# permon/permon

Measured on NVIDIA B200. Metric: mpgp_iterations_per_second, higher is better.
Workload: dtype f64

## Files before the change

### permon_b200/csrc/kernels.cu

```cuda
#include <climits>
#include <cuda_runtime.h>
#include <nvtx3/nvToolsExt.h>
#include <stdarg.h>
#include <stddef.h>
#include <stdio.h>
#include <string.h>
#include <time.h>

#include <algorithm>
#include <string>
#include <type_traits>
#include <utility>
#include <vector>

#include "device.h"

namespace pb {

static DevCtx      g_ctx;
int                g_p2p_size = 1;
static std::string g_err;
DevCtx            &ctx() { return g_ctx; }
const char        *last_error() { return g_err.c_str(); }

// ... 1137 lines not shown
  if (warp == PK_CT / 32) {
    int pidn = 0;
    if (blockIdx.x < ntiles) pidn = __ldg(A.st_pid + tile_at(blockIdx.x, ord.ta, ord.tb, rev));
    int      s = 0, filled = 0;
    uint32_t ph = 0;
    for (int i = blockIdx.x; i < ntiles; i += gridDim.x) {
      const int tile = tile_at(i, ord.ta, ord.tb, rev);
      const int pid = pidn;
      const int ni = i + gridDim.x;
      if (ni < ntiles) pidn = __ldg(A.st_pid + tile_at(ni, ord.ta, ord.tb, rev));
      if (filled >= nstages) mbar_wait(&empty_bar[s], ph ^ 1u);
      else filled++;
      unsigned char   *st = stages + (size_t)s * stage_bytes;
      const StPattern *P = reinterpret_cast<const StPattern *>(smem_raw) + pid;
      const int        r0 = tile * TR, r1 = min(r0 + TR, A.n);
      const bool       fullt = (r1 - r0 == TR) && vec_tma;
      bool             windowed = fullt && win_ok;
      uint32_t         wbytes = 0;
      const int        nwin = P->nwin;
      for (int w = 0; w < nwin; w++) {
        const int lo = r0 + P->wlo[w];
        if (lo < 0 || lo + P->wlen[w] > A.ncols) windowed = false;
        wbytes += (uint32_t)P->wlen[w] * 8u;
      }
      if (lane == 0) {
        reinterpret_cast<int *>(st)[0] = pid;
        reinterpret_cast<int *>(st)[1] = windowed ? 1 : 0;
      }
      if (fullt) {
        if (lane == 0) {
          mbar_arrive_expect_tx(&full_bar[s], (uint32_t)TR + (uint32_t)nv * TR * 8u + (windowed ? wbytes : 0u));
          bulk_g2s(st + ST_MASK_OFF, A.st_masks + r0, (uint32_t)TR, &full_bar[s]);
          if (windowed)
            for (int w = 0; w < nwin; w++) bulk_g2s(st + ST_WIN_OFF + (size_t)w * PB_ST_WCAP, x + (r0 + P->wlo[w]), (uint32_t)P->wlen[w] * 8u, &full_bar[s]);
          for (int v = 0; v < nv; v++) bulk_g2s(st + vec_off + (size_t)v * TR * 8, epi.vsrc(v) + r0, (uint32_t)TR * 8u, &full_bar[s]);
        }
      } else {
        for (int t = lane; t < TR; t += 32) st[ST_MASK_OFF + t] = (t < r1 - r0) ? __ldg(A.st_masks + r0 + t) : (unsigned char)0;
        for (int v = 0; v < nv; v++) {
          double       *vs = (double *)(st + vec_off) + (size_t)v * TR;
          const double *src = epi.vsrc(v) + r0;
          for (int t = lane; t < r1 - r0; t += 32) vs[t] = src[t];
        }
        fence_proxy_async_smem();
        __syncwarp();
        if (lane == 0) mbar_arrive(&full_bar[s]);
      }
      if (++s == nstages) {
        s = 0;
        ph ^= 1u;
      }
    }
  } else {
    const uint32_t smem_a = smem_u32(smem_raw), stages_a = smem_a + (uint32_t)pats_bytes;
    int            s = 0;
    uint32_t       ph = 0;
    for (int i = blockIdx.x; i < ntiles; i += gridDim.x) {
      const int tile = tile_at(i, ord.ta, ord.tb, rev);
      mbar_wait(&full_bar[s], ph);
      const uint32_t st_a = stages_a + (uint32_t)s * (uint32_t)stage_bytes;
      const uint32_t vs_a = st_a + (uint32_t)vec_off + 8u * threadIdx.x;
      const uint32_t pid = (uint32_t)lds_s32(st_a), windowed = (uint32_t)lds_s32(st_a + 4u);
      const uint32_t P_a = smem_a + pid * (uint32_t)sizeof(StPattern);
      const uint32_t L = (uint32_t)lds_s32(P_a);
      const uint32_t m0 = lds_u8(st_a + ST_MASK_OFF + threadIdx.x), m1 = lds_u8(st_a + ST_MASK_OFF + threadIdx.x + PK_CT);
      const int      r0 = tile * TR + threadIdx.x, r1 = r0 + PK_CT;
      double         s0, s1;
      if (windowed) st_win2_dispatch(L, m0, m1, P_a, st_a + ST_WIN_OFF + 8u * threadIdx.x, gx, s0, s1);
      else st_row2_dispatch(L, m0, m1, P_a + (uint32_t)offsetof(StPattern, v), P_a + (uint32_t)offsetof(StPattern, d), gx, r0, r1, s0, s1);
      if (r0 < A.n) epi.row_s(r0, vs_a, s0, acc);
      if (r1 < A.n) epi.row_s(r1, vs_a + PK_CT * 8u, s1, acc);
      __syncwarp();
      if (lane == 0) mbar_arrive(&empty_bar[s]);
      if (++s == nstages) {
        s = 0;
        ph ^= 1u;
      }
    }
  }
  epi.finalize(acc);
}


template <int LMAX, class G>
__device__ __forceinline__ double sd_row(int L, uint32_t m, const StPattern &P, const G &gx, int r)
{
  constexpr uint32_t FULL = (1u << LMAX) - 1u;
  const char        *xr = reinterpret_cast<const char *>(gx.x + r);
  if (__all_sync(0xffffffffu, L == LMAX && m == FULL)) {
    double xv[LMAX];
    int    db[LMAX];
#pragma unroll
    for (int j = 0; j < LMAX; j++) db[j] = P.d[j] * 8;
#pragma unroll
    for (int j = 0; j < LMAX; j++) xv[j] = gx.ld(reinterpret_cast<const double *>(xr + (long long)db[j]));
    __syncwarp();
    double s = 0.0;
#pragma unroll
    for (int j = 0; j < LMAX; j++) s += P.v[j] * xv[j];
    return s;
  }
  double xv[LMAX], vv[LMAX];
#pragma unroll
  for (int j = 0; j < LMAX; j++) {
    const bool on = (j < L) && ((m >> j) & 1u);
    xv[j]         = on ? gx.ld(reinterpret_cast<const double *>(xr + (long long)(P.d[j] * 8))) : 0.0;
  }
  __syncwarp();
#pragma unroll
  for (int j = 0; j < LMAX; j++) vv[j] = P.v[j];
  double s = 0.0;
#pragma unroll
  for (int j = 0; j < LMAX; j++)
    if ((j < L) && ((m >> j) & 1u)) s += vv[j] * xv[j];
  return s;
}

__device__ __forceinline__ void l2_prefetch_bulk(const double *p, long long e0, long long e1, long long n)
{
  if (e0 < 0) e0 = 0;
  if (e1 > n) e1 = n;
  uintptr_t a0 = (uintptr_t)(p + e0), a1 = (uintptr_t)(p + e1);
  a0 = (a0 + 15) & ~(uintptr_t)15;
  a1 &= ~(uintptr_t)15;
  if (a1 > a0) asm volatile("cp.async.bulk.prefetch.L2.global [%0], %1;" ::"l"(a0), "r"((uint32_t)(a1 - a0)) : "memory");
}
template <class Epi>
__device__ __forceinline__ void sd_prefetch_tile(const Epi &epi, const double *gx, int tile, int rows, int n, int ncols, bool rev, const TileOrder &ord, int lane)
{
  const long long r0 = (long long)tile * rows;
  const int       nv = epi.nvec();
  if (lane == 0) {
    const int d = rev ? ord.dlo : ord.dhi;
    l2_prefetch_bulk(gx, r0 + d, r0 + d + rows, ncols);
  } else if (lane <= nv) {
    const double *v = epi.vsrc(lane - 1);
    if (v != gx) l2_prefetch_bulk(v, r0, r0 + rows, n);
  }
}

template <class Epi, int LMAX, int MINB>
__global__ void __launch_bounds__(NT, MINB) k_spmv_sd(CsrDev A, const double *__restrict__ x, Epi epi, TileOrder ord)
{
  pdl_enter();
  if (!epi.active()) return;
  __shared__ StPattern s_pats[PB_ST_MAXPAT];
  {
    const int  nw = A.st_npat * (int)(sizeof(StPattern) / 4);
    const int *src = reinterpret_cast<const int *>(A.st_pats);
    int       *dst = reinterpret_cast<int *>(s_pats);
    for (int k = threadIdx.x; k < nw; k += NT) dst[k] = __ldg(src + k);
  }
  __syncthreads();
  const int  ntiles = (A.n + TR - 1) / TR;
  const bool rev = epi.reverse();
  const typename Epi::Gather gx = epi.gather(x);
  typename Epi::Acc acc;
  epi.init(acc);
  uint32_t m_next = 0;
  int      pid_next = 0;
  if ((int)blockIdx.x < ntiles) {
    const int t0 = tile_at(blockIdx.x, ord.ta, ord.tb, rev);
    pid_next = __ldg(A.st_pid + t0);
    m_next   = __ldg(A.st_masks + (size_t)t0 * TR + threadIdx.x);
  }
  for (int i = blockIdx.x; i < ntiles; i += gridDim.x) {
    const int      tile = tile_at(i, ord.ta, ord.tb, rev);
    const uint32_t m = m_next;
    const int      pid = pid_next;
    const int      ni = i + gridDim.x;
    const int      r = tile * TR + threadIdx.x;
    const bool     live = r < A.n;
    if (ord.pf > 0 && threadIdx.x < 32) {
      const long long pi = (long long)i + (long long)ord.pf * gridDim.x;
      if (pi < ntiles) sd_prefetch_tile(epi, gx.x, tile_at((int)pi, ord.ta, ord.tb, rev), TR, A.n, A.ncols, rev, ord, (int)threadIdx.x);
    }
    const typename Epi::Pre pre = epi.preload(live ? r : 0);
    if (ni < ntiles) {
      const int tn = tile_at(ni, ord.ta, ord.tb, rev);
      pid_next = __ldg(A.st_pid + tn);
      m_next   = __ldg(A.st_masks + (size_t)tn * TR + threadIdx.x);
    }
    const StPattern &P = s_pats[pid];
    const double     sum = sd_row<LMAX>(P.L, m, P, gx, r);
    if (live) epi.row_p(r, sum, pre, acc);
  }
  epi.finalize(acc);
}


template <int LMAX, class G>
__device__ __forceinline__ void sd_row2(int L, uint32_t m0, uint32_t m1, const StPattern &P, const G &gx, int r, double &s0, double &s1)
{
  constexpr uint32_t FULL = (1u << LMAX) - 1u;
  const char        *xr = reinterpret_cast<const char *>(gx.x + r);
  double             x0[LMAX], x1[LMAX], vv[LMAX];
  if (__all_sync(0xffffffffu, L == LMAX && m0 == FULL && m1 == FULL)) {
#pragma unroll
    for (int j = 0; j < LMAX; j++) {
      const double *a = reinterpret_cast<const double *>(xr + (long long)(P.d[j] * 8));
      x0[j]           = gx.ld(a);
      x1[j]           = gx.ld(a + 1);
    }
    __syncwarp();
#pragma unroll
    for (int j = 0; j < LMAX; j++) vv[j] = P.v[j];
    s0 = 0.0;
    s1 = 0.0;
#pragma unroll
    for (int j = 0; j < LMAX; j++) s0 += vv[j] * x0[j];
#pragma unroll
    for (int j = 0; j < LMAX; j++) s1 += vv[j] * x1[j];
    return;
  }
#pragma unroll
  for (int j = 0; j < LMAX; j++) {
    const double *a = reinterpret_cast<const double *>(xr + (long long)(P.d[j] * 8));
    const bool    on0 = (j < L) && ((m0 >> j) & 1u), on1 = (j < L) && ((m1 >> j) & 1u);
    x0[j]             = on0 ? gx.ld(a) : 0.0;
    x1[j]             = on1 ? gx.ld(a + 1) : 0.0;
  }
  __syncwarp();
#pragma unroll
  for (int j = 0; j < LMAX; j++) vv[j] = P.v[j];
  s0 = 0.0;
  s1 = 0.0;
#pragma unroll
  for (int j = 0; j < LMAX; j++)
    if ((j < L) && ((m0 >> j) & 1u)) s0 += vv[j] * x0[j];
#pragma unroll
  for (int j = 0; j < LMAX; j++)
    if ((j < L) && ((m1 >> j) & 1u)) s1 += vv[j] * x1[j];
}

template <class Epi, int LMAX, int MINB>
__global__ void __launch_bounds__(NT, MINB) k_spmv_sd2(CsrDev A, const double *__restrict__ x, Epi epi, TileOrder ord)
{
  pdl_enter();
  if (!epi.active()) return;
  __shared__ StPattern s_pats[PB_ST_MAXPAT];
  {
    const int  nw = A.st_npat * (int)(sizeof(StPattern) / 4);
    const int *src = reinterpret_cast<const int *>(A.st_pats);
    int       *dst = reinterpret_cast<int *>(s_pats);
    for (int k = threadIdx.x; k < nw; k += NT) dst[k] = __ldg(src + k);
  }
  __syncthreads();
  const int  nst = (A.n + 2 * TR - 1) / (2 * TR);
  const int  half = threadIdx.x >> 7;
  const bool rev = epi.reverse();
  const typename Epi::Gather gx = epi.gather(x);
  typename Epi::Acc acc;
  epi.init(acc);
  uchar2 m_next = make_uchar2(0, 0);
  int    pid_next = 0;
  if ((int)blockIdx.x < nst) {
    const int t0 = tile_at(blockIdx.x, ord.ta, ord.tb, rev);
    pid_next = __ldg(A.st_pid + 2 * t0 + half);
    m_next   = __ldg(reinterpret_cast<const uchar2 *>(A.st_masks + (size_t)t0 * (2 * TR)) + threadIdx.x);
  }
  for (int i = blockIdx.x; i < nst; i += gridDim.x) {
    const int    st = tile_at(i, ord.ta, ord.tb, rev);
    const uchar2 m = m_next;
    const int    pid = pid_next;
    const int    ni = i + gridDim.x;
    const int    r = st * (2 * TR) + 2 * (int)threadIdx.x;
    const bool   live = r < A.n;
    const typename Epi::Pre2 pre = epi.preload2(live ? r : 0);
// ... 276 lines not shown
    }
    static size_t attr_smem = 0;
    if (smem > attr_smem) {
      cudaFuncSetAttribute(k_spmv_st<Epi>, cudaFuncAttributeMaxDynamicSharedMemorySize, (int)smem);
      attr_smem = smem;
    }
    static int    occ = 0;
    static size_t occ_smem = (size_t)-1;
    if (!occ || occ_smem != smem) {
      int nb = 0;
      if (cudaOccupancyMaxActiveBlocksPerMultiprocessor(&nb, k_spmv_st<Epi>, PK_CT + 32, smem) != cudaSuccess || nb < 1) nb = 1;
      occ      = nb;
      occ_smem = smem;
    }
    int ntiles = (A.n + TR - 1) / TR, grid = g_ctx.sm_count * occ;
    if (grid > ntiles) grid = ntiles;
    if (grid > max_red_blocks()) grid = max_red_blocks();
    if (ord.tb <= ord.ta || ord.tb > ntiles) {
      ord.ta = 0;
      ord.tb = ntiles;
    }
    launch_k(k_spmv_st<Epi>, grid, PK_CT + 32, smem, A, x, epi, nstages, (int)stage, pats_bytes, win_ok, vec_tma, ord);
    return 0;
  }
}


template <class Epi, int LMAX>
static int launch_sd_l(const CsrDev &A, const double *x, const Epi &epi, TileOrder ord)
{
  static int pairs = -1;
  if (pairs < 0) {
    const char *e = getenv("PERMON_B200_SD_PAIRS");
    pairs = (e && e[0] == '1') ? 1 : 0;
  }
  if (pairs && (A.n % 2 == 0) && aligned16(x) && epi.pair_ok()) {
    auto       k2 = k_spmv_sd2<Epi, LMAX, 4>;
    static int occ2 = 0;
    if (!occ2) {
      int nb = 0;
      if (cudaOccupancyMaxActiveBlocksPerMultiprocessor(&nb, k2, NT, 0) != cudaSuccess || nb < 1) nb = 1;
      occ2 = nb;
    }
    const int ntiles = (A.n + TR - 1) / TR, nst = (ntiles + 1) / 2;
    int       grid = g_ctx.sm_count * occ2;
    if (grid > nst) grid = nst;
    if (grid > max_red_blocks()) grid = max_red_blocks();
    TileOrder o2;
    o2.ta = (ord.ta + 1) / 2;
    o2.tb = ord.tb / 2;
    if (o2.tb <= o2.ta || o2.tb > nst || ord.tb <= ord.ta || ord.tb > ntiles || (ord.ta == 0 && ord.tb == ntiles)) {
      o2.ta = 0;
      o2.tb = nst;
    }
    launch_k(k2, grid, NT, 0, A, x, epi, o2);
    return 0;
  }
  auto kern = k_spmv_sd<Epi, LMAX, 5>;
  static int pf = -1;
  if (pf < 0) {
    const char *e = getenv("PERMON_B200_SD_PF");
    pf = e ? atoi(e) : 0;
    if (pf < 0 || pf > 64) pf = 0;
  }
  ord.pf  = pf;
  ord.dlo = A.st_dlo;
  ord.dhi = A.st_dhi;
  static int occ = 0;
  if (!occ) {
    int nb = 0;
    if (cudaOccupancyMaxActiveBlocksPerMultiprocessor(&nb, kern, NT, 0) != cudaSuccess || nb < 1) nb = 1;
    occ = nb;
  }
  int ntiles = (A.n + TR - 1) / TR, grid = g_ctx.sm_count * occ;
  if (grid > ntiles) grid = ntiles;
  if (grid > max_red_blocks()) grid = max_red_blocks();
  if (ord.tb <= ord.ta || ord.tb > ntiles) {
    ord.ta = 0;
    ord.tb = ntiles;
  }
  launch_k(kern, grid, NT, 0, A, x, epi, ord);
  return 0;
}
template <class Epi>
static int launch_sd(const CsrDev &A, const double *x, const Epi &epi, TileOrder ord)
{
  switch (A.st_lmax) {
  case 3: return launch_sd_l<Epi, 3>(A, x, epi, ord);
  case 5: return launch_sd_l<Epi, 5>(A, x, epi, ord);
  case 7: return launch_sd_l<Epi, 7>(A, x, epi, ord);
  default: return launch_sd_l<Epi, 8>(A, x, epi, ord);
  }
}

template <class Epi>
static int launch_spmv(const CsrDev &A, const double *x, const Epi &epi, int family, double bytes, TileOrder ord = TileOrder())
{
  prof_pre(family, bytes);
  if (A.n == 0) {
    k_spmv_vector<Epi, 32><<<1, NT, 0, g_ctx.stream>>>(A, x, epi);
  } else if (A.kind == 5) {
    launch_ell(A, x, epi);
  } else if (A.kind == 4) {
    static int direct = -1;
    if (direct < 0) {
      const char *e = getenv("PERMON_B200_ST_KERNEL");
      direct = (e && !strcmp(e, "windows")) ? 0 : 1;
    }
    if (direct) PB_CHK(launch_sd(A, x, epi, ord));
    else PB_CHK(launch_st(A, x, epi, ord));
  } else if (A.kind == 3) {
    PB_CHK(launch_pk(A, x, epi, ord));
  } else if (A.kind == 2) {
    launch_tma(A, x, epi);
  } else if (A.kind == 0) {
    static int    occ = 0;
    static size_t occ_smem = (size_t)-1;
    size_t        smem = (size_t)A.tile_cap * sizeof(double);
    if (!occ || occ_smem != smem) {
      occ      = occ_blocks(k_spmv_stream<Epi>, smem);
      occ_smem = smem;
    }
    int ntiles = (A.n + TR - 1) / TR;
    int grid   = g_ctx.sm_count * occ;
    if (grid > ntiles) grid = ntiles;
    if (grid > max_red_blocks()) grid = max_red_blocks();
    k_spmv_stream<Epi><<<grid, NT, smem, g_ctx.stream>>>(A, x, epi);
  } else {
    switch (A.W) {
    case 2: launch_vector<Epi, 2>(A, x, epi); break;
    case 4: launch_vector<Epi, 4>(A, x, epi); break;
    case 8: launch_vector<Epi, 8>(A, x, epi); break;
    case 16: launch_vector<Epi, 16>(A, x, epi); break;
    default: launch_vector<Epi, 32>(A, x, epi); break;
    }
  }
  prof_post(family);
  LAUNCH_CHECK();
  return 0;
}

double csr_stream_bytes(const CsrDev &A)
{
  if (A.kind == 3 || A.kind == 4) return (double)A.pk_bytes;
  if (A.kind == 5) return 12.0 * (double)A.ell_elems + 4.0 * A.n;
  return 12.0 * (double)A.nnz + 4.0 * (A.n + 1);
}

void spmv_stats(int n, const int *h_ia, int *maxrow_out, int *cap_out)
{
  int maxrow = 0, cap = 0;
  for (int r0 = 0; r0 < n; r0 += TR) {
    int r1 = (r0 + TR < n) ? r0 + TR : n;
    int t  = h_ia[r1] - h_ia[r0];
    if (t > cap) cap = t;
  }
#pragma omp parallel for reduction(max : maxrow) schedule(static)
  for (int r = 0; r < n; r++) {
    int l = h_ia[r + 1] - h_ia[r];
    if (l > maxrow) maxrow = l;
  }
  *maxrow_out = maxrow;
  *cap_out    = cap;
}
int spmv_config(CsrDev &A, const int *h_ia)
{
  int maxrow, cap;
  spmv_stats(A.n, h_ia, &maxrow, &cap);
  spmv_decide(A, maxrow, cap);
  return 0;
}
void spmv_decide(CsrDev &A, int maxrow, int cap)
{
  const int n = A.n;
  const double avg = n ? (double)A.nnz / n : 0.0;
  const char  *force = getenv("PERMON_B200_SPMV");
  bool         stream = (cap <= 5632 && maxrow <= 64);
  if (force && !strcmp(force, "vector")) stream = false;
  if (stream) {
    A.kind     = 2;
    if ((force && !strcmp(force, "stream")) || A.rows) A.kind = 0;
    A.tile_cap = (cap + 3 + 31) & ~31;
    if (A.tile_cap < 32) A.tile_cap = 32;
    const char *st = getenv("PERMON_B200_STAGES");
    A.stages = st ? atoi(st) : 2;
  } else {
    A.kind = 1;
    int W  = 32;
    if (avg <= 3) W = 2;
    else if (avg <= 6) W = 4;
    else if (avg <= 12) W = 8;
    else if (avg <= 24) W = 16;
    A.W = W;
  }
}

struct EpiPlain {
  typedef GatherPlain Gather;
  __device__ Gather gather(const double *x) const { return Gather{x}; }
  double *y;
  int     accumulate;
  struct Acc {};
  __device__ bool active() const { return true; }
  __device__ bool reverse() const { return false; }
  __device__ void init(Acc &) const {}
  __device__ void row(int r, double ax, Acc &) const { y[r] = accumulate ? y[r] + ax : ax; }
  struct Pre {};
  __device__ Pre preload(int) const { return Pre{}; }
  __device__ void row_p(int r, double ax, const Pre &, Acc &a) const { row(r, ax, a); }
  __device__ void finalize(Acc &) const {}
  __host__ __device__ int  nvec() const { return 0; }
  __host__ __device__ const double *vsrc(int) const { return nullptr; }
  int nvec_host() const { return nvec(); }
  const double *vsrc_host(int i) const { return vsrc(i); }
  __device__ void row_s(int r, uint32_t, double ax, Acc &a) const { row(r, ax, a); }

  struct Pre2 {};
  __device__ Pre2 preload2(int) const { return Pre2{}; }
  __device__ void row2_p(int r, double a0, double a1, const Pre2 &, Acc &a) const
  {
    row(r, a0, a);
    row(r + 1, a1, a);
  }
  bool pair_ok() const { return true; }
};

struct EpiGated {
  typedef GatherPlain Gather;
  __device__ Gather gather(const double *x) const { return Gather{x}; }
  double        *y;
  const MpgpCtl *S;
  int            phase;
  struct Acc {};
  __device__ bool active() const
  {
    if (S->reason != 0) return false;
    return phase == 0 ? true : (S->step == 'e' || S->init);
  }
  __device__ bool reverse() const { return false; }
  __device__ void init(Acc &) const {}
  __device__ void row(int r, double ax, Acc &) const { y[r] = ax; }
  struct Pre {};
  __device__ Pre preload(int) const { return Pre{}; }
  __device__ void row_p(int r, double ax, const Pre &, Acc &a) const { row(r, ax, a); }
  struct Pre2 {};
  __device__ Pre2 preload2(int) const { return Pre2{}; }
  __device__ void row2_p(int r, double a0, double a1, const Pre2 &, Acc &a) const
  {
    row(r, a0, a);
    row(r + 1, a1, a);
  }
  bool pair_ok() const { return true; }
  __device__ void finalize(Acc &) const {}
  __host__ __device__ int  nvec() const { return 0; }
  __host__ __device__ const double *vsrc(int) const { return nullptr; }
  int nvec_host() const { return nvec(); }
  const double *vsrc_host(int i) const { return vsrc(i); }
  __device__ void row_s(int r, uint32_t, double ax, Acc &a) const { row(r, ax, a); }
};

struct AccRed {
  double v[PB_NRED];
  int    halo_ok;
};

struct GhostRet {
  double ax;
  int    ok;
};
__device__ __noinline__ GhostRet ghost_slow(const GhostMerge &gm, int r, double ax, int halo_ok)
{
  GhostRet  out{ax, halo_ok};
  const int k = __ldg(gm.row_map + (r < gm.lo ? r : r - gm.hi + gm.lo));
  if (k < 0) return out;
  if (!halo_ok) {
    for (int q = 0; q < gm.nflags; q++) wait_flag(gm.flags + (size_t)q * PB_FLAG_STRIDE, gm.seq);
    out.ok = 1;
  }
  const int e0 = __ldg(gm.oia + k), e1 = __ldg(gm.oia + k + 1);
  for (int e = e0; e < e1; e++) out.ax += __ldg(gm.oa + e) * __ldcg(gm.ghost + __ldg(gm.oja + e));
  return out;
}
__device__ __forceinline__ double ghost_apply(const GhostMerge &gm, int r, double ax, int &halo_ok)
{
  if (gm.row_map == nullptr || (r >= gm.lo && r < gm.hi)) return ax;
  const GhostRet g = ghost_slow(gm, r, ax, halo_ok);
  halo_ok = g.ok;
  return g.ax;
}

template <int MODE, bool GHOST>
struct EpiAT {
  typedef GatherPlain Gather;
  __device__ Gather gather(const double *x) const { return Gather{x}; }
  const double        *p, *x;
  double              *Ap;
  BoxDev               bx;
  const double        *B;
  int                  m, n;
  const MpgpCtl       *S;
  RedBuf               rb;
  GhostMerge           gm;
  typedef AccRed       Acc;
  __device__ bool active() const { return S->reason == 0; }
  __device__ bool reverse() const { return S->sweep != 0; }
  __device__ void init(Acc &a) const
  {
#pragma unroll
    for (int k = 0; k < PB_NRED; k++) a.v[k] = 0.0;
    a.v[RA_FEAS] = HUGE_VAL;
    a.halo_ok    = 0;
  }
  __device__ void row(int r, double ax, Acc &a) const
  {
    if constexpr (GHOST) ax = ghost_apply(gm, r, ax, a.halo_ok);
    Ap[r] = ax;
    const double pr = __ldg(p + r);
    a.v[RA_PAP] += pr * ax;
    if constexpr (MODE != 0) {
      BoxVal b;
      b.has_lb = true;
      b.has_ub = (MODE == 2);
      b.lb     = __ldg(bx.lb + r);
      b.ub     = (MODE == 2) ? __ldg(bx.ub + r) : 0.0;
      a.v[RA_FEAS] = box_feas_lazy(__ldg(x + r), pr, b, a.v[RA_FEAS]);
    } else {
#pragma unroll
      for (int j = 0; j < PB_MAXEQ; j++)
        if (j < m) a.v[RA_BP + j] += B[(size_t)j * n + r] * pr;
      a.v[RA_FEAS] = box_feas_lazy(x[r], pr, load_box(bx, r), a.v[RA_FEAS]);
    }
  }
  struct Pre {
    double p, x, lb, ub;
  };
  __device__ Pre preload(int r) const
  {
    Pre q;
    q.p  = __ldg(p + r);
    q.x  = __ldg(x + r);
    q.lb = (MODE != 0 || bx.lb) ? __ldg(bx.lb + r) : 0.0;
    q.ub = (MODE == 2 || (MODE == 0 && bx.ub)) ? __ldg(bx.ub + r) : 0.0;
    return q;
  }
  __device__ void row_p(int r, double ax, const Pre &q, Acc &a) const
  {
    if constexpr (GHOST) ax = ghost_apply(gm, r, ax, a.halo_ok);
    Ap[r] = ax;
    a.v[RA_PAP] += q.p * ax;
    BoxVal b;
    b.has_lb = (MODE != 0) || bx.lb != nullptr;
    b.has_ub = (MODE == 2) || (MODE == 0 && bx.ub != nullptr);
    b.lb     = q.lb;
    b.ub     = q.ub;
    if constexpr (MODE == 0) {
#pragma unroll
      for (int j = 0; j < PB_MAXEQ; j++)
        if (j < m) a.v[RA_BP + j] += B[(size_t)j * n + r] * q.p;
    }
    a.v[RA_FEAS] = box_feas_lazy(q.x, q.p, b, a.v[RA_FEAS]);
  }
  struct Pre2 {
    double2 p, x, lb, ub;
  };
  __device__ Pre2 preload2(int r) const
  {
    Pre2 q;
    q.p  = __ldg(reinterpret_cast<const double2 *>(p + r));
    q.x  = __ldg(reinterpret_cast<const double2 *>(x + r));
    q.lb = (MODE != 0 || bx.lb) ? __ldg(reinterpret_cast<const double2 *>(bx.lb + r)) : make_double2(0.0, 0.0);
    q.ub = (MODE == 2 || (MODE == 0 && bx.ub)) ? __ldg(reinterpret_cast<const double2 *>(bx.ub + r)) : make_double2(0.0, 0.0);
    return q;
  }
  __device__ void row2_p(int r, double a0, double a1, const Pre2 &q, Acc &a) const
  {
    if constexpr (GHOST) {
      a0 = ghost_apply(gm, r, a0, a.halo_ok);
      a1 = ghost_apply(gm, r + 1, a1, a.halo_ok);
    }
    *reinterpret_cast<double2 *>(Ap + r) = make_double2(a0, a1);
    a.v[RA_PAP] += q.p.x * a0;
    a.v[RA_PAP] += q.p.y * a1;
    BoxVal b0, b1;
    b0.has_lb = b1.has_lb = (MODE != 0) || bx.lb != nullptr;
    b0.has_ub = b1.has_ub = (MODE == 2) || (MODE == 0 && bx.ub != nullptr);
    b0.lb = q.lb.x; b1.lb = q.lb.y;
    b0.ub = q.ub.x; b1.ub = q.ub.y;
    if constexpr (MODE == 0) {
#pragma unroll
      for (int j = 0; j < PB_MAXEQ; j++)
        if (j < m) {
          a.v[RA_BP + j] += B[(size_t)j * n + r] * q.p.x;
          a.v[RA_BP + j] += B[(size_t)j * n + r + 1] * q.p.y;
        }
    }
    a.v[RA_FEAS] = box_feas_lazy(q.x.x, q.p.x, b0, a.v[RA_FEAS]);
    a.v[RA_FEAS] = box_feas_lazy(q.x.y, q.p.y, b1, a.v[RA_FEAS]);
  }
  bool pair_ok() const { return aligned16(p) && aligned16(x) && aligned16(Ap) && aligned16(bx.lb) && aligned16(bx.ub); }
  __device__ void finalize(Acc &a) const { grid_reduce8<(1 << RA_FEAS)>(a.v, rb, nullptr); }
  __host__ __device__ int nvec() const { return 2 + (bx.lb ? 1 : 0) + (bx.ub ? 1 : 0) + m; }
  int nvec_host() const { return nvec(); }
  const double *vsrc_host(int i) const { return vsrc(i); }
  __host__ __device__ const double *vsrc(int i) const
  {
    if (i == 0) return p;
    if (i == 1) return x;
    int k = 2;
    if (bx.lb) {
      if (i == k) return bx.lb;
      k++;
    }
    if (bx.ub) {
      if (i == k) return bx.ub;
      k++;
    }
    return B + (size_t)(i - k) * n;
  }
  __device__ void row_s(int r, uint32_t va, double ax, Acc &a) const
  {
    if constexpr (GHOST) ax = ghost_apply(gm, r, ax, a.halo_ok);
    Ap[r] = ax;
    const double pr = lds_f64(va);
    a.v[RA_PAP] += pr * ax;
    const double xr = lds_f64(va + TR * 8);
    if constexpr (MODE != 0) {
      BoxVal b;
      b.has_lb = true;
      b.has_ub = (MODE == 2);
      b.lb     = lds_f64(va + 2 * TR * 8);
      b.ub     = (MODE == 2) ? lds_f64(va + 3 * TR * 8) : 0.0;
      a.v[RA_FEAS] = box_feas_lazy(xr, pr, b, a.v[RA_FEAS]);
    } else {
      BoxVal   b;
      uint32_t k = 2;
      b.has_lb = bx.lb != nullptr;
      b.has_ub = bx.ub != nullptr;
      b.lb     = b.has_lb ? lds_f64(va + (k++) * TR * 8) : 0.0;
      b.ub     = b.has_ub ? lds_f64(va + (k++) * TR * 8) : 0.0;
#pragma unroll
      for (int j = 0; j < PB_MAXEQ; j++)
        if (j < m) a.v[RA_BP + j] += lds_f64(va + (k + j) * TR * 8) * pr;
      a.v[RA_FEAS] = box_feas_lazy(xr, pr, b, a.v[RA_FEAS]);
    }
  }
};

template <int MODE, bool GHOST>
struct EpiA2T {
  typedef GatherPlain Gather;
  __device__ Gather gather(const double *x) const { return Gather{x}; }
  const double        *x, *b;
  double              *g, *p;
  BoxDev               bx;
  const double        *B;
  int                  m, n;
  const MpgpCtl       *S;
  RedBuf               rb;
  GhostMerge           gm;
  typedef AccRed       Acc;
  __device__ bool active() const { return S->reason == 0 && (S->step == 'e' || S->init); }
  __device__ bool reverse() const { return S->sweep != 0; }
  __device__ void init(Acc &a) const
  {
#pragma unroll
    for (int k = 0; k < PB_NRED; k++) a.v[k] = 0.0;
    a.halo_ok = 0;
  }
  __device__ void row(int r, double ax, Acc &a) const
  {
    double gr = ax;
    if constexpr (GHOST) gr = ghost_apply(gm, r, ax, a.halo_ok);
    BoxVal bv;
    if constexpr (MODE != 0) {
      bv.has_lb = true;
      bv.has_ub = (MODE == 2);
      bv.lb     = __ldg(bx.lb + r);
      bv.ub     = (MODE == 2) ? __ldg(bx.ub + r) : 0.0;
    } else {
      bv = load_box(bx, r);
      if (m > 0) {
        double t = 0.0;
        for (int j = 0; j < m; j++) t += B[(size_t)j * n + r] * S->Bu[j];
        gr += S->rho * t;
      }
    }
    gr -= __ldg(b + r);
    double gf, gc;
    box_split(x[r], gr, bv, bx.astol, gf, gc);
    g[r] = gr;
    p[r] = gf;
    const double gP = gf + gc;
    a.v[RB_GP2] += gP * gP;
    a.v[RB_GC2] += gc * gc;
    a.v[RB_GF2] += gf * gf;
  }
  struct Pre {
    double x, b, lb, ub;
  };
  __device__ Pre preload(int r) const
  {
    Pre q;
    q.x  = __ldg(x + r);
    q.b  = __ldg(b + r);
    q.lb = (MODE != 0 || bx.lb) ? __ldg(bx.lb + r) : 0.0;
    q.ub = (MODE == 2 || (MODE == 0 && bx.ub)) ? __ldg(bx.ub + r) : 0.0;
    return q;
  }
  __device__ void row_p(int r, double ax, const Pre &q, Acc &a) const
  {
    double gr = ax;
    if constexpr (GHOST) gr = ghost_apply(gm, r, ax, a.halo_ok);
    BoxVal bv;
    bv.has_lb = (MODE != 0) || bx.lb != nullptr;
    bv.has_ub = (MODE == 2) || (MODE == 0 && bx.ub != nullptr);
    bv.lb     = q.lb;
    bv.ub     = q.ub;
    if constexpr (MODE == 0) {
      if (m > 0) {
        double t = 0.0;
        for (int j = 0; j < m; j++) t += B[(size_t)j * n + r] * S->Bu[j];
        gr += S->rho * t;
      }
    }
    gr -= q.b;
    double gf, gc;
    box_split(q.x, gr, bv, bx.astol, gf, gc);
    g[r] = gr;
    p[r] = gf;
    const double gP = gf + gc;
    a.v[RB_GP2] += gP * gP;
    a.v[RB_GC2] += gc * gc;
    a.v[RB_GF2] += gf * gf;
// ... 26 lines not shown
      if (m > 0) {
        double t0 = 0.0, t1 = 0.0;
        for (int j = 0; j < m; j++) {
          t0 += B[(size_t)j * n + r] * S->Bu[j];
          t1 += B[(size_t)j * n + r + 1] * S->Bu[j];
        }
        gr0 += S->rho * t0;
        gr1 += S->rho * t1;
      }
    }
    gr0 -= q.b.x;
    gr1 -= q.b.y;
    double gf0, gc0, gf1, gc1;
    box_split(q.x.x, gr0, b0, bx.astol, gf0, gc0);
    box_split(q.x.y, gr1, b1, bx.astol, gf1, gc1);
    *reinterpret_cast<double2 *>(g + r) = make_double2(gr0, gr1);
    *reinterpret_cast<double2 *>(p + r) = make_double2(gf0, gf1);
    const double gP0 = gf0 + gc0, gP1 = gf1 + gc1;
    a.v[RB_GP2] += gP0 * gP0;
    a.v[RB_GC2] += gc0 * gc0;
    a.v[RB_GF2] += gf0 * gf0;
    a.v[RB_GP2] += gP1 * gP1;
    a.v[RB_GC2] += gc1 * gc1;
    a.v[RB_GF2] += gf1 * gf1;
  }
  bool pair_ok() const { return aligned16(x) && aligned16(b) && aligned16(g) && aligned16(p) && aligned16(bx.lb) && aligned16(bx.ub); }
  __device__ void finalize(Acc &a) const { grid_reduce8<0>(a.v, rb, nullptr); }
  __host__ __device__ int nvec() const { return 2 + (bx.lb ? 1 : 0) + (bx.ub ? 1 : 0) + m; }
  int nvec_host() const { return nvec(); }
  const double *vsrc_host(int i) const { return vsrc(i); }
  __host__ __device__ const double *vsrc(int i) const
  {
    if (i == 0) return x;
    if (i == 1) return b;
    int k = 2;
    if (bx.lb) {
      if (i == k) return bx.lb;
      k++;
    }
    if (bx.ub) {
      if (i == k) return bx.ub;
      k++;
    }
    return B + (size_t)(i - k) * n;
  }
  __device__ void row_s(int r, uint32_t va, double ax, Acc &a) const
  {
    BoxVal bv;
    double gr = ax;
    if constexpr (GHOST) gr = ghost_apply(gm, r, ax, a.halo_ok);
    if constexpr (MODE != 0) {
      bv.has_lb = true;
      bv.has_ub = (MODE == 2);
      bv.lb     = lds_f64(va + 2 * TR * 8);
      bv.ub     = (MODE == 2) ? lds_f64(va + 3 * TR * 8) : 0.0;
    } else {
      uint32_t k = 2;
      bv.has_lb = bx.lb != nullptr;
      bv.has_ub = bx.ub != nullptr;
      bv.lb     = bv.has_lb ? lds_f64(va + (k++) * TR * 8) : 0.0;
      bv.ub     = bv.has_ub ? lds_f64(va + (k++) * TR * 8) : 0.0;
      if (m > 0) {
        double tt = 0.0;
#pragma unroll
        for (int j = 0; j < PB_MAXEQ; j++)
          if (j < m) tt += lds_f64(va + (k + j) * TR * 8) * S->Bu[j];
        gr += S->rho * tt;
      }
    }
    gr -= lds_f64(va + TR * 8);
    double gf, gc;
    box_split(lds_f64(va), gr, bv, bx.astol, gf, gc);
    g[r] = gr;
    p[r] = gf;
    const double gP = gf + gc;
    a.v[RB_GP2] += gP * gP;
    a.v[RB_GC2] += gc * gc;
    a.v[RB_GF2] += gf * gf;
  }
};

struct EpiPower {
  typedef GatherScaled Gather;
  const double *w;
  double        s;
  double       *y;
  RedBuf        rb;
  __device__ Gather gather(const double *x) const { return Gather{x, s}; }
  typedef AccRed Acc;
  __device__ bool active() const { return true; }
  __device__ bool reverse() const { return false; }
  __device__ void init(Acc &a) const
  {
#pragma unroll
    for (int k = 0; k < PB_NRED; k++) a.v[k] = 0.0;
    a.halo_ok = 0;
  }
  __device__ void row(int r, double ax, Acc &a) const
  {
    y[r] = ax;
    const double vr = w[r] * s;
    a.v[0] += ax * vr;
    a.v[1] += vr * vr;
  }
  struct Pre {
    double w;
  };
  __device__ Pre preload(int r) const { return Pre{__ldg(w + r)}; }
  __device__ void row_p(int r, double ax, const Pre &q, Acc &a) const
  {
    y[r] = ax;
    const double vr = q.w * s;
    a.v[0] += ax * vr;
    a.v[1] += vr * vr;
  }
  struct Pre2 {
    double2 w;
  };
  __device__ Pre2 preload2(int r) const { return Pre2{__ldg(reinterpret_cast<const double2 *>(w + r))}; }
  __device__ void row2_p(int r, double a0, double a1, const Pre2 &q, Acc &a) const
  {
    *reinterpret_cast<double2 *>(y + r) = make_double2(a0, a1);
    const double v0 = q.w.x * s, v1 = q.w.y * s;
    a.v[0] += a0 * v0;
    a.v[1] += v0 * v0;
    a.v[0] += a1 * v1;
    a.v[1] += v1 * v1;
  }
  bool pair_ok() const { return aligned16(w) && aligned16(y); }
  __device__ void finalize(Acc &a) const { grid_reduce8<0>(a.v, rb, nullptr); }
  __host__ __device__ int nvec() const { return 1; }
  __host__ __device__ const double *vsrc(int) const { return w; }
  int nvec_host() const { return 1; }
  const double *vsrc_host(int) const { return w; }
  __device__ void row_s(int r, uint32_t va, double ax, Acc &a) const
  {
    y[r] = ax;
    const double vr = lds_f64(va) * s;
    a.v[0] += ax * vr;
    a.v[1] += vr * vr;
  }
};
int k_power_step(const CsrDev &A, const double *w, double s, double *y, RedBuf rb)
{
  if (A.kind != 3 && A.kind != 4) {
    set_error("internal: fused power step needs a packed matrix");
    return 76;
  }
  EpiPower e{w, s, y, rb};
  return launch_spmv(A, w, e, KF_SPMV_PLAIN, csr_stream_bytes(A) + 16.0 * A.n);
}

int k_spmv(const CsrDev &A, const double *x, double *y, int accumulate)
{
  EpiPlain e{y, accumulate};
  return launch_spmv(A, x, e, KF_SPMV_PLAIN, csr_stream_bytes(A) + 16.0 * A.n);
}

int k_spmv_gated(const CsrDev &A, const double *x, double *y, const MpgpCtl *S, int phase)
{
  EpiGated e{y, S, phase};
  return launch_spmv(A, x, e, KF_SPMV_PLAIN, csr_stream_bytes(A) + 16.0 * A.n);
}

static double bytes_A(const CsrDev &A, const MpgpVecs &v)
{
// ... 769 lines not shown
```

Baseline: 354.0.

## Add plane-marching stencil SpMV kernel reusing x values across far-diagonal tiles

Adds a new SpMV kernel for the stencil/diagonal format in which each block walks a column of tiles separated by the largest diagonal offset D. It keeps the x values at offsets -D, 0 and +D in registers as a sliding window, so each x element is loaded about once instead of three times across the far diagonals. The kernel is enabled by default when D is a multiple of the tile size and the epilogue has no ghost merge. In exchange, parallelism drops to tp*nseg work items, extra loads occur at segment boundaries, and the kernel carries more register state and a fixed occupancy bound.

```diff
diff --git a/permon_b200/csrc/kernels.cu b/permon_b200/csrc/kernels.cu
--- a/permon_b200/csrc/kernels.cu
+++ b/permon_b200/csrc/kernels.cu
@@ -1243,6 +1243,26 @@
 }
 
 
+template <int LMAX>
+__device__ __forceinline__ double sd_sum_full(const StPattern &P, const double (&xv)[LMAX])
+{
+  double s = 0.0;
+#pragma unroll
+  for (int j = 0; j < LMAX; j++) s += P.v[j] * xv[j];
+  return s;
+}
+template <int LMAX>
+__device__ __forceinline__ double sd_sum_masked(int L, uint32_t m, const StPattern &P, const double (&xv)[LMAX])
+{
+  double vv[LMAX];
+#pragma unroll
+  for (int j = 0; j < LMAX; j++) vv[j] = P.v[j];
+  double s = 0.0;
+#pragma unroll
+  for (int j = 0; j < LMAX; j++)
+    if ((j < L) && ((m >> j) & 1u)) s += vv[j] * xv[j];
+  return s;
+}
 template <int LMAX, class G>
 __device__ __forceinline__ double sd_row(int L, uint32_t m, const StPattern &P, const G &gx, int r)
 {
@@ -1256,25 +1276,16 @@
 #pragma unroll
     for (int j = 0; j < LMAX; j++) xv[j] = gx.ld(reinterpret_cast<const double *>(xr + (long long)db[j]));
     __syncwarp();
-    double s = 0.0;
-#pragma unroll
-    for (int j = 0; j < LMAX; j++) s += P.v[j] * xv[j];
-    return s;
-  }
-  double xv[LMAX], vv[LMAX];
+    return sd_sum_full<LMAX>(P, xv);
+  }
+  double xv[LMAX];
 #pragma unroll
   for (int j = 0; j < LMAX; j++) {
     const bool on = (j < L) && ((m >> j) & 1u);
     xv[j]         = on ? gx.ld(reinterpret_cast<const double *>(xr + (long long)(P.d[j] * 8))) : 0.0;
   }
   __syncwarp();
-#pragma unroll
-  for (int j = 0; j < LMAX; j++) vv[j] = P.v[j];
-  double s = 0.0;
-#pragma unroll
-  for (int j = 0; j < LMAX; j++)
-    if ((j < L) && ((m >> j) & 1u)) s += vv[j] * xv[j];
-  return s;
+  return sd_sum_masked<LMAX>(L, m, P, xv);
 }
 
 __device__ __forceinline__ void l2_prefetch_bulk(const double *p, long long e0, long long e1, long long n)
@@ -1345,6 +1356,129 @@
     const StPattern &P = s_pats[pid];
     const double     sum = sd_row<LMAX>(P.L, m, P, gx, r);
     if (live) epi.row_p(r, sum, pre, acc);
+  }
+  epi.finalize(acc);
+}
+
+
+struct SdMarch {
+  int tp = 0;
+  int nplanes = 0;
+  int seg = 0;
+  int nseg = 0;
+};
+
+template <int LMAX, class G>
+__device__ __forceinline__ double sdm_row(int L, uint32_t m, bool canon, const StPattern &P, const G &gx, int r, int D, double xm, double xc, double xp)
+{
+  constexpr uint32_t FULL = (1u << LMAX) - 1u;
+  const char        *xr = reinterpret_cast<const char *>(gx.x + r);
+  double             xv[LMAX];
+  if (__all_sync(0xffffffffu, canon && m == FULL)) {
+#pragma unroll
+    for (int j = 0; j < LMAX; j++) {
+      if (j == 0) xv[j] = xm;
+      else if (j == LMAX / 2) xv[j] = xc;
+      else if (j == LMAX - 1) xv[j] = xp;
+      else xv[j] = gx.ld(reinterpret_cast<const double *>(xr + (long long)(P.d[j] * 8)));
+    }
+    __syncwarp();
+    return sd_sum_full<LMAX>(P, xv);
+  }
+#pragma unroll
+  for (int j = 0; j < LMAX; j++) {
+    const bool on = (j < L) && ((m >> j) & 1u);
+    const int  d = P.d[j];
+    double     v = 0.0;
+    if (d == -D) v = xm;
+    else if (d == 0) v = xc;
+    else if (d == D) v = xp;
+    else if (on) v = gx.ld(reinterpret_cast<const double *>(xr + (long long)(d * 8)));
+    xv[j] = on ? v : 0.0;
+  }
+  __syncwarp();
+  return sd_sum_masked<LMAX>(L, m, P, xv);
+}
+
+template <class Epi, int LMAX, int MINB>
+__global__ void __launch_bounds__(NT, MINB) k_spmv_sdm(CsrDev A, const double *__restrict__ x, Epi epi, SdMarch mp)
+{
+  pdl_enter();
+  if (!epi.active()) return;
+  __shared__ StPattern s_pats[PB_ST_MAXPAT];
+  {
+    const int  nw = A.st_npat * (int)(sizeof(StPattern) / 4);
+    const int *src = reinterpret_cast<const int *>(A.st_pats);
+    int       *dst = reinterpret_cast<int *>(s_pats);
+    for (int k = threadIdx.x; k < nw; k += NT) dst[k] = __ldg(src + k);
+  }
+  __syncthreads();
+  const int D = mp.tp * TR;
+  uint32_t  canon;
+  {
+    const int lane = threadIdx.x & 31;
+    bool      c = false;
+    if (lane < A.st_npat) {
+      const StPattern &P = s_pats[lane];
+      c = P.L == LMAX && P.d[0] == -D && P.d[LMAX / 2] == 0 && P.d[LMAX - 1] == D;
+    }
+    canon = __ballot_sync(0xffffffffu, c);
+  }
+  const int  ntiles = (A.n + TR - 1) / TR;
+  const bool rev = epi.reverse();
+  const int  dq = rev ? -1 : 1;
+  const long long step = rev ? -(long long)D : (long long)D;
+  const typename Epi::Gather gx = epi.gather(x);
+  typename Epi::Acc acc;
+  epi.init(acc);
+  auto ldx = [&](long long i) { return (i >= 0 && i < (long long)A.ncols) ? gx.ld(gx.x + i) : 0.0; };
+  const int nitems = mp.tp * mp.nseg;
+  for (int i = blockIdx.x; i < nitems; i += gridDim.x) {
+    const int k = rev ? nitems - 1 - i : i;
+    const int sg = k / mp.tp, col = k - sg * mp.tp;
+    int       q0 = sg * mp.seg, q1 = q0 + mp.seg;
+    if (q1 > mp.nplanes) q1 = mp.nplanes;
+    const int qt = (ntiles - 1 - col) / mp.tp + 1;
+    if (q1 > qt) q1 = qt;
+    const int nq = q1 - q0;
+    if (nq <= 0) continue;
+    int               t = (rev ? q1 - 1 : q0) * mp.tp + col;
+    double            xb, xc, xa;
+    uint32_t          m;
+    int               pid;
+    typename Epi::Pre pre;
+    {
+      const int r = t * TR + (int)threadIdx.x;
+      xb = ldx(r - step);
+      xc = ldx(r);
+      xa = ldx(r + step);
+      m   = __ldg(A.st_masks + (size_t)t * TR + threadIdx.x);
+      pid = __ldg(A.st_pid + t);
+      pre = epi.preload(r < A.n ? r : 0);
+    }
+    for (int s = 0; s < nq; s++) {
+      const int  r = t * TR + (int)threadIdx.x;
+      const bool more = s + 1 < nq;
+      const int  tn = t + dq * mp.tp, rn = tn * TR + (int)threadIdx.x;
+      const double lead = more ? ldx(rn + step) : 0.0;
+      uint32_t     mn = 0;
+      int          pidn = 0;
+      if (more) {
+        mn   = __ldg(A.st_masks + (size_t)tn * TR + threadIdx.x);
+        pidn = __ldg(A.st_pid + tn);
+      }
+      const typename Epi::Pre pren = epi.preload(more && rn < A.n ? rn : 0);
+      const StPattern &P = s_pats[pid];
+      const double     sum = sdm_row<LMAX>(P.L, m, (canon >> pid) & 1u, P, gx, r, D, rev ? xa : xb, xc, rev ? xb : xa);
+      if (r < A.n) epi.row_p(r, sum, pre, acc);
+      xb  = xc;
+      xc  = xa;
+      xa  = lead;
+      m   = mn;
+      pid = pidn;
+      pre = pren;
+      t   = tn;
+    }
   }
   epi.finalize(acc);
 }
@@ -1787,9 +1921,59 @@
   launch_k(kern, grid, NT, 0, A, x, epi, ord);
   return 0;
 }
+static constexpr int SDM_MINB = 4;
+
 template <class Epi>
-static int launch_sd(const CsrDev &A, const double *x, const Epi &epi, TileOrder ord)
-{
+static SdMarch sd_march_plan(const CsrDev &A)
+{
+  SdMarch    mp;
+  static int sw = -1;
+  if (sw < 0) {
+    const char *e = getenv("PERMON_B200_SD_MARCH");
+    sw = e ? atoi(e) : 1;
+    if (sw < 0) sw = 1;
+  }
+  const int D = -A.st_dlo > A.st_dhi ? -A.st_dlo : A.st_dhi;
+  if (Epi::ghost || sw == 0 || D % TR != 0 || D / TR < 2) return mp;
+  const int ntiles = (A.n + TR - 1) / TR;
+  mp.tp      = D / TR;
+  mp.nplanes = (ntiles + mp.tp - 1) / mp.tp;
+  const int grid = g_ctx.sm_count * SDM_MINB;
+  int       nseg = (16 * grid + mp.tp - 1) / mp.tp;
+  if (sw >= 2) nseg = (mp.nplanes + sw - 1) / sw;
+  if (nseg > mp.nplanes) nseg = mp.nplanes;
+  if (nseg < 1) nseg = 1;
+  mp.seg  = (mp.nplanes + nseg - 1) / nseg;
+  mp.nseg = (mp.nplanes + mp.seg - 1) / mp.seg;
+  return mp;
+}
+static double sdm_extra_bytes(const SdMarch &mp) { return mp.tp ? 16.0 * TR * mp.tp * (mp.nseg - 1) : 0.0; }
+
+template <class Epi, int LMAX>
+static int launch_sdm_l(const CsrDev &A, const double *x, const Epi &epi, const SdMarch &mp)
+{
+  auto       kern = k_spmv_sdm<Epi, LMAX, SDM_MINB>;
+  const int  nitems = mp.tp * mp.nseg;
+  int        grid = g_ctx.sm_count * SDM_MINB;
+  if (grid > nitems) grid = nitems;
+  if (grid > max_red_blocks()) grid = max_red_blocks();
+  launch_k(kern, grid, NT, 0, A, x, epi, mp);
+  return 0;
+}
+
+template <class Epi>
+static int launch_sd(const CsrDev &A, const double *x, const Epi &epi, TileOrder ord, const SdMarch &mp)
+{
+  if constexpr (!Epi::ghost) {
+    if (mp.tp) {
+      switch (A.st_lmax) {
+      case 3: return launch_sdm_l<Epi, 3>(A, x, epi, mp);
+      case 5: return launch_sdm_l<Epi, 5>(A, x, epi, mp);
+      case 7: return launch_sdm_l<Epi, 7>(A, x, epi, mp);
+      default: return launch_sdm_l<Epi, 8>(A, x, epi, mp);
+      }
+    }
+  }
   switch (A.st_lmax) {
   case 3: return launch_sd_l<Epi, 3>(A, x, epi, ord);
   case 5: return launch_sd_l<Epi, 5>(A, x, epi, ord);
@@ -1801,18 +1985,20 @@
 template <class Epi>
 static int launch_spmv(const CsrDev &A, const double *x, const Epi &epi, int family, double bytes, TileOrder ord = TileOrder())
 {
-  prof_pre(family, bytes);
+  static int direct = -1;
+  if (direct < 0) {
+    const char *e = getenv("PERMON_B200_ST_KERNEL");
+    direct = (e && !strcmp(e, "windows")) ? 0 : 1;
+  }
+  SdMarch mp;
+  if (A.kind == 4 && A.n > 0 && direct) mp = sd_march_plan<Epi>(A);
+  prof_pre(family, bytes + sdm_extra_bytes(mp));
   if (A.n == 0) {
     k_spmv_vector<Epi, 32><<<1, NT, 0, g_ctx.stream>>>(A, x, epi);
   } else if (A.kind == 5) {
     launch_ell(A, x, epi);
   } else if (A.kind == 4) {
-    static int direct = -1;
-    if (direct < 0) {
-      const char *e = getenv("PERMON_B200_ST_KERNEL");
-      direct = (e && !strcmp(e, "windows")) ? 0 : 1;
-    }
-    if (direct) PB_CHK(launch_sd(A, x, epi, ord));
+    if (direct) PB_CHK(launch_sd(A, x, epi, ord, mp));
     else PB_CHK(launch_st(A, x, epi, ord));
   } else if (A.kind == 3) {
     PB_CHK(launch_pk(A, x, epi, ord));
@@ -1902,6 +2088,7 @@
 
 struct EpiPlain {
   typedef GatherPlain Gather;
+  static constexpr bool ghost = false;
   __device__ Gather gather(const double *x) const { return Gather{x}; }
   double *y;
   int     accumulate;
@@ -1932,6 +2119,7 @@
 
 struct EpiGated {
   typedef GatherPlain Gather;
+  static constexpr bool ghost = false;
   __device__ Gather gather(const double *x) const { return Gather{x}; }
   double        *y;
   const MpgpCtl *S;
@@ -1997,6 +2185,7 @@
 template <int MODE, bool GHOST>
 struct EpiAT {
   typedef GatherPlain Gather;
+  static constexpr bool ghost = GHOST;
   __device__ Gather gather(const double *x) const { return Gather{x}; }
   const double        *p, *x;
   double              *Ap;
@@ -2154,6 +2343,7 @@
 template <int MODE, bool GHOST>
 struct EpiA2T {
   typedef GatherPlain Gather;
+  static constexpr bool ghost = GHOST;
   __device__ Gather gather(const double *x) const { return Gather{x}; }
   const double        *x, *b;
   double              *g, *p;
@@ -2346,6 +2536,7 @@
 
 struct EpiPower {
   typedef GatherScaled Gather;
+  static constexpr bool ghost = false;
   const double *w;
   double        s;
   double       *y;
diff --git a/profiles/sd_march_ab.py b/profiles/sd_march_ab.py
--- /dev/null
+++ b/profiles/sd_march_ab.py
@@ -0,0 +1,74 @@
+import argparse
+import json
+import os
+import subprocess
+import sys
+import tempfile
+
+import numpy as np
+
+ROOT = os.path.dirname(os.path.dirname(os.path.abspath(__file__)))
+
+
+def card():
+    try:
+        q = subprocess.run(["nvidia-smi", "--query-gpu=name,power.limit,clocks.max.sm", "--format=csv,noheader"], capture_output=True, text=True, timeout=60)
+        return q.stdout.strip()
+    except Exception as e:
+        return f"unknown ({e})"
+
+
+def one(workload, steps, setting, dump_dir):
+    env = {k: v for k, v in os.environ.items() if k != "PERMON_B200_SD_MARCH"}
+    if setting != "default":
+        env["PERMON_B200_SD_MARCH"] = setting
+    cmd = [sys.executable, os.path.join(ROOT, "bench.py"), "--gpus", "1", "--workload", workload, "--steps", str(steps), "--no-e2e",
+           "--no-cpu-baseline", "--no-parity", "--dump-outputs", dump_dir]
+    p = subprocess.run(cmd, env=env, capture_output=True, text=True, timeout=1800, cwd=ROOT)
+    if p.returncode != 0:
+        raise SystemExit(f"bench.py failed ({workload}, {steps}, {setting}):\n{p.stdout[-2000:]}\n{p.stderr[-3000:]}")
+    line = json.loads([s for s in p.stdout.splitlines() if s.startswith("{")][-1])
+    pk = line["roofline"]["per_kernel"]
+    x = np.load(os.path.join(dump_dir, f"{workload}_x.npy"))
+    return dict(value=line["value"], ms_per_step=line["ms_per_step"], step_mix=line["details"]["step_mix"],
+                kernels_ms={k: v["avg_ms"] for k, v in pk.items()}), x
+
+
+def main():
+    ap = argparse.ArgumentParser()
+    ap.add_argument("out")
+    ap.add_argument("--runs", default="c3:20,c2:20,c3:2000")
+    ap.add_argument("--reps", type=int, default=3)
+    ap.add_argument("--settings", default="default,0")
+    a = ap.parse_args()
+    settings = a.settings.split(",")
+    summary = dict(card=card(), settings=settings, runs={})
+    for spec in a.runs.split(","):
+        wl, steps = spec.split(":")
+        res = {s: [] for s in settings}
+        x_ref = None
+        maxrel = {s: 0.0 for s in settings}
+        for rep in range(a.reps):
+            for s in settings:
+                with tempfile.TemporaryDirectory() as d:
+                    r, x = one(wl, int(steps), s, d)
+                if x_ref is None:
+                    x_ref = x
+                maxrel[s] = max(maxrel[s], float(np.linalg.norm(x - x_ref) / np.linalg.norm(x_ref)))
+                res[s].append(r)
+                print(wl, steps, s, rep, r["value"], r["kernels_ms"], r["step_mix"], flush=True)
+        entry = {}
+        for s in settings:
+            v = [r["value"] for r in res[s]]
+            km = {k: [r["kernels_ms"].get(k) for r in res[s]] for k in res[s][0]["kernels_ms"]}
+            entry[s] = dict(values=v, mean=float(np.mean(v)), spread=float(max(v) - min(v)), kernels_ms=km,
+                            kernels_ms_mean={k: float(np.mean([t for t in vs if t is not None])) for k, vs in km.items()},
+                            step_mixes=[r["step_mix"] for r in res[s]], relx_vs_first_run=maxrel[s])
+        summary["runs"][spec] = entry
+        with open(a.out, "w") as f:
+            json.dump(summary, f, indent=1)
+    print(json.dumps(summary, indent=1))
+
+
+if __name__ == "__main__":
+    main()
```

After: 240.8, median of 6. 32.0% lower.
